# chenxuhao/GraphMiner

Hardware: AMD Instinct MI355X
Metric: million edges processed/sec + total match count (higher is better)
Workload: dtype int32 (vertex ids, offsets; uint64 counts); 1 GPU; tc: triangle counting, LiveJournal stand-in; graph=rmat_s22_ef10_seed42, nv=4194304, ne_sym=81171116, tasks=40585558, max_degree=777, parallelism=task-chunk round-robin x1, replicated CSR

## Files before the change

### graphminer_amd/csrc/gm_graph.hip

```cpp
#include "gm_host.h"
#include <unordered_map>
#include "gm_scan.h"
#include "gm_setops.h"
using namespace gm;

thread_local std::string g_last_error;
thread_local TempPool *g_temp_pool = nullptr;

namespace {
std::mutex g_opt_mu;
std::list<std::pair<std::string, std::string>> g_opts;
}
const char *gm_opt(const char *name) {
  if (!name) return nullptr;
  {
    std::lock_guard<std::mutex> lk(g_opt_mu);
    for (const auto &kv : g_opts)
      if (kv.first == name) return kv.second.c_str();
  }
#ifdef GM_DEVEL
  return getenv(name);
#else
  return nullptr;
#endif
// ... 165 lines not shown
  *n = 0;
  int c = 0;
  hipError_t e = hipGetDeviceCount(&c);
  if (e != hipSuccess) return hip_fail(e, "hipGetDeviceCount", __FILE__, __LINE__);
  *n = c;
  return c > 0 ? GM_OK : GM_ERR_NO_DEVICE;
}

extern "C" int gm_graph_setup_times(const gm_graph *g, gm_setup_times *out) {
  if (!g || !out) return GM_ERR_INVALID;
  *out = g->setup;
  for (const gm_graph *r : {g->dag_cache, g->relabel_cache[0], g->relabel_cache[1], g->relabel_cache[2]})
    if (r) {
      gm_setup_times t;
      const int rc = gm_graph_setup_times(r, &t);
      if (rc) return rc;
      out->orient_ms += t.orient_ms;
      out->table_ms += t.table_ms;
      out->bitmap_ms += t.bitmap_ms;
      out->relabel_ms += t.relabel_ms;
      out->other_ms += t.other_ms;
    }
  return GM_OK;
}
extern "C" void gm_graph_free(gm_graph *g) {
  if (!g) return;
  if (g->dag_cache) gm_graph_free(g->dag_cache);
  g->dag_cache = nullptr;
  for (auto &r : g->relabel_cache) {
    if (r) gm_graph_free(r);
    r = nullptr;
  }
  (void)hipSetDevice(g->device);
  free_tables(g);
  for (auto &b : g->bitmap_sets) {
    if (b.d_bitmaps) dev_free(b.d_bitmaps);
    if (b.d_row_slot) dev_free(b.d_row_slot);
  }
  if (g->d_rp) dev_free(g->d_rp);
  if (g->d_rp64) dev_free(g->d_rp64);
  if (g->own_col && g->d_col) dev_free(g->d_col);
  if (g->d_edesc) dev_free(g->d_edesc);
  if (g->d_symdeg) dev_free(g->d_symdeg);
  if (g->d_trp) dev_free(g->d_trp);
  if (g->d_tdesc) dev_free(g->d_tdesc);
  if (g->d_tedge) dev_free(g->d_tedge);
  for (void *q : {(void *)g->d_emoff, (void *)g->d_tmoff, (void *)g->d_smask, (void *)g->d_sup_far_rows})
    if (q) dev_free(q);
  if (g->d_long_rows) dev_free(g->d_long_rows);
  if (g->d_long_prefix) dev_free(g->d_long_prefix);
  if (g->d_colk) dev_free(g->d_colk);
  if (g->d_tdesck) dev_free(g->d_tdesck);
  if (g->d_kst) dev_free(g->d_kst);
  for (void *q : {(void *)g->d_kst_et, (void *)g->d_tedgel, (void *)g->d_kst2, (void *)g->d_tdescl2})
    if (q) dev_free(q);
  if (g->d_kst_rp) dev_free(g->d_kst_rp);
  if (g->d_trpl) dev_free(g->d_trpl);
  if (g->d_tdescl) dev_free(g->d_tdescl);
  if (g->d_sup) dev_free(g->d_sup);
  for (void *q : {(void *)g->d_w5sup, (void *)g->d_w5ed, (void *)g->d_w5deg, (void *)g->d_w5tv2, (void *)g->d_w5out})
    if (q) dev_free(q);
  for (void *q : {(void *)g->d_s6e1, (void *)g->d_wrect_mask, (void *)g->d_wrect_tasks})
    if (q) dev_free(q);
  for (void *q : {(void *)g->d_newid, (void *)g->d_lsup, (void *)g->d_lent, (void *)g->d_lrev, (void *)g->d_lmark, (void *)g->d_lfront, (void *)g->d_ltruss,
                  (void *)g->d_lcnt, (void *)g->d_list_off})
    if (q) dev_free(q);
  free_clique_plans(g);
  if (g->d_wide_mat) dev_free(g->d_wide_mat);
  if (g->d_wide_sorted) dev_free(g->d_wide_sorted);
  if (g->d_wide_queue) dev_free(g->d_wide_queue);
  for (auto &st_ : g->aux_stream) if (st_) (void)hipStreamDestroy(st_);
  for (auto &ev_ : g->aux_done) if (ev_) (void)hipEventDestroy(ev_);
  if (g->pool.base) dev_free(g->pool.base);
  if (g->d_counters) dev_free(g->d_counters);
  if (g->d_scratch) dev_free(g->d_scratch);
  if (g->d_core) dev_free(g->d_core);
  for (void *q : {(void *)g->d_cg_tri, (void *)g->d_cg_rowbase, (void *)g->d_cg_bid, (void *)g->d_cg_blk})
    if (q) dev_free(q);
  if (g->d_csym) dev_free(g->d_csym);
  if (g->d_cfirst) dev_free(g->d_cfirst);
  if (g->d_idx0) dev_free(g->d_idx0);
  if (g->d_wblock_prefix) dev_free(g->d_wblock_prefix);
  if (g->d_house_prefix) dev_free(g->d_house_prefix);
  if (g->d_pent_touched) dev_free(g->d_pent_touched);
  if (g->d_house_t) dev_free(g->d_house_t);
  if (g->d_house_tlt) dev_free(g->d_house_tlt);
  if (g->d_house_tasks) dev_free(g->d_house_tasks);
  if (g->d_house_acc) dev_free(g->d_house_acc);
  if (g->d_house_touched) dev_free(g->d_house_touched);
  if (g->d_house_bnd) dev_free(g->d_house_bnd);
  if (g->d_house_lds_tasks) dev_free(g->d_house_lds_tasks);
  if (g->d_house_cut_tasks) dev_free(g->d_house_cut_tasks);
  if (g->d_rect_tasks) dev_free(g->d_rect_tasks);
  if (g->d_rect_bnd) dev_free(g->d_rect_bnd);
  if (g->d_rect_lds_tasks) dev_free(g->d_rect_lds_tasks);
  if (g->d_rect_cut_tasks) dev_free(g->d_rect_cut_tasks);
  if (g->d_rect_acc) dev_free(g->d_rect_acc);
  for (auto &pr : g->ev)
    for (auto &e : pr)
      if (e) (void)hipEventDestroy(e);
  const bool last = g->counted && dev_handle_died(g->device);
  delete g;
  if (last) big_cache_trim();
}

int finish_handle(gm_graph *g) {
  if (!g->counted) {
// ... 971 lines not shown
```

### graphminer_amd/csrc/gm_host.h

```cpp
#pragma once
#include "../../include/graphminer_amd.h"
#include "gm_mine.h"
#include "gm_setops.h"

#include <algorithm>
#include <chrono>
#include <cstdio>
#include <cstring>
#include <list>
#include <mutex>
#include <string>
#include <thread>
#include <vector>

using namespace gm;

extern thread_local std::string g_last_error;
extern thread_local int g_last_hip_error;
int hip_fail(hipError_t e, const char *what, const char *file, int line);
#define HIP_TRY(call)                                              \
  do {                                                             \
    hipError_t _e = (call);                                        \
    if (_e != hipSuccess) return hip_fail(_e, #call, __FILE__, __LINE__); \
  } while (0)
// ... 150 lines not shown
struct CliquePlan {
  int rank = 0, world = 1, policy = 0, target = 0, order_which = 1;
  int stage = 1024;
  bool topo = false;
  ChunkTable *tabN = nullptr;
  long long n_first = 0, n_step = 1, n_count = 0;
  const int *d_order = nullptr;
  std::vector<int> verts;
  int *d_verts = nullptr;
  unsigned long long *d_slot_base = nullptr;
  int *d_mcls_slots = nullptr;
  int4 *d_mcls_rec = nullptr;
  int core_base = -1;
  std::vector<CliqueRound> rounds;
  unsigned long long wide_edges = 0;
};

struct BitmapSet {
  int min_deg = 0;
  RowFilter rf;
  unsigned *d_bitmaps = nullptr;
  int *d_row_slot = nullptr;
  size_t n = 0;
  unsigned long long words = 0;
};

struct gm_graph {
  int device = 0;
  int nv = 0;
  long long ne = 0;
  int max_deg = 0;
  int *d_rp = nullptr;
  long long *d_rp64 = nullptr;
  int *d_col = nullptr;
  bool own_col = true;
  int *d_symdeg = nullptr;
  int2 *d_edesc = nullptr;
  int *d_trp = nullptr;
  int2 *d_tdesc = nullptr;
  int *d_tedge = nullptr;
  int *d_colk = nullptr;
  int2 *d_tdesck = nullptr;
  unsigned long long n_inline_keys = 0;
  unsigned *d_kst = nullptr;
  int kst_state = 0;
  int n_long_tasks = 0;
  int *d_kst_rp = nullptr;
  int *d_trpl = nullptr;
  int2 *d_tdescl = nullptr;
  int2 *d_kst_et = nullptr;
  int *d_tedgel = nullptr;
  unsigned *d_kst2 = nullptr;
  int2 *d_tdescl2 = nullptr;
  int kst_lmax = 0;
  int *d_long_rows = nullptr;
  long long *d_long_prefix = nullptr;
  int n_long_rows = -1;
  long long long_edges = 0;
  unsigned *d_sup = nullptr;
  unsigned *d_w5sup = nullptr, *d_w5ed = nullptr;
  int *d_w5deg = nullptr;
  unsigned long long *d_w5tv2 = nullptr, *d_w5out = nullptr;
  bool w5_tri = false, w5_vert = false;
  unsigned *d_s6e1 = nullptr;
  unsigned long long *d_wrect_mask = nullptr;
  int2 *d_wrect_tasks = nullptr;
  unsigned long long n_wrect_tasks = 0;
  int wrect_range = 0, wrect_grp = 1;
  bool wrect_ready = false;
  int *d_newid = nullptr;
  unsigned *d_lsup = nullptr;
  unsigned *d_lent = nullptr;
  int *d_lrev = nullptr;
  bool lrev_ready = false;
  unsigned char *d_lmark = nullptr;
  int *d_lfront = nullptr;
  unsigned *d_ltruss = nullptr;
  unsigned *d_lcnt = nullptr;
  unsigned long long *d_list_off = nullptr;
  unsigned long long list_total = 0;
  bool list_ready = false;
  unsigned *d_emoff = nullptr, *d_tmoff = nullptr;
  unsigned long long *d_smask = nullptr;
  unsigned long long smask_words = 0;
  int *d_sup_far_rows = nullptr;
  int n_sup_far_rows = 0;
  int smask_min_tail = 0;
  int smask_state = 0;
  std::vector<int> h_rp;
  std::list<ChunkTable> tables;
  unsigned long long *d_counters = nullptr;
  unsigned *d_scratch = nullptr;
  size_t scratch_bytes = 0;
  static constexpr int kEvRing = 64;
  hipEvent_t ev[kEvRing][4] = {};
  bool ev_corner[kEvRing] = {};
  unsigned long long ev_launches = 0;
  int cu_count = 256;
  gm_graph *dag_cache = nullptr;
  gm_graph *relabel_cache[3] = {nullptr, nullptr, nullptr};
  int sorted_state = 0;
  int topo_state = 0;
  unsigned long long giant_edges = ~0ull;
  double tri_per_edge = -1.0;
  double mean_sq_deg = -1.0;
  bool topo_relabel_failed = false;
// ... 201 lines not shown
```

### graphminer_amd/csrc/gm_launch.hip

```cpp
#include "gm_host.h"

using namespace gm;

enum FinMode : int { FIN_COPY = 0, FIN_MOTIF3 = 1, FIN_MOTIF3_FORMULA = 2, FIN_RAW4 = 3, FIN_HALF_SIGNED = 4 };

__host__ __device__ static inline int finalize_math(int mode, unsigned long long base, const unsigned long long *c, unsigned long long *out) {
  if (mode == FIN_MOTIF3) {
    out[0] = c[2] - c[0];
    out[1] = c[1];
  } else if (mode == FIN_MOTIF3_FORMULA) {
    out[0] = base - 3ull * c[0];
    out[1] = c[0];
  } else if (mode == FIN_RAW4) {
    out[0] = c[0]; out[1] = c[1]; out[2] = c[2]; out[3] = c[3];
  } else if (mode == FIN_HALF_SIGNED) {
    out[0] = (unsigned long long)((long long)c[0] >> 1);
  } else {
    out[0] = c[0];
  }
  return mode == FIN_RAW4 ? 4 : (mode == FIN_MOTIF3 || mode == FIN_MOTIF3_FORMULA) ? 2 : 1;
}

__global__ void finalize_kernel(int mode, unsigned long long base, const unsigned long long *__restrict__ c,
                                unsigned long long *__restrict__ out) {
// ... 314 lines not shown
    q.count = (int)so->n;
    q.order = so->d;
    r.my_edges += so->edges;
    return GM_OK;
  }
  if (la->policy == GM_PART_VERTEX) {
    if (int rcv = table_host_views(g, tb)) return rcv;
    const long long vlo = (long long)g->nv * rank / world, vhi = (long long)g->nv * (rank + 1) / world;
    auto first_chunk_at = [&](long long v) {
      long long lo = 0, hi = n;
      while (lo < hi) {
        const long long mid = (lo + hi) / 2;
        if (tb->first_vertex[(size_t)mid] < v) lo = mid + 1; else hi = mid;
      }
      return lo;
    };
    first = first_chunk_at(vlo);
    count = first_chunk_at(vhi) - first;
  } else {
    gm_partition((int64_t)n, rank, world, la->policy, (int64_t *)&first, (int64_t *)&step, (int64_t *)&count);
  }
  q.first = (int)first;
  q.step = (int)step;
  q.count = (int)count;
  if (first == 0 && step == 1 && count == n) { r.my_edges += tb->total_edges; return GM_OK; }
  if (int rcv = table_host_views(g, tb)) return rcv;
  if (step == 1) r.my_edges += tb->edge_prefix[first + count] - tb->edge_prefix[first];
  else for (long long j = first; j < n; j += step) {
    const size_t c = lpt ? (size_t)tb->order[which][(size_t)j] : (size_t)j;
    r.my_edges += tb->edge_prefix[c + 1] - tb->edge_prefix[c];
  }
  return GM_OK;
}

static int fill_mine_params(PatternRun &r, int k) {
  gm_graph *g = r.ctx.g;
  const gm_launch *la = &r.ctx.la;
  const PatternPlan &pl = r.pl;
  MineParams &p = r.p;
  memset(&p, 0, sizeof p);
  p.g = graph_view(g);
  if (int rc = ensure_edesc(g)) return rc;
  p.g.edesc = g->d_edesc;
  if (pl.use_tct) {
    p.g.trp = g->d_trp;
    p.g.tdesc = g->d_tdesc;
    p.g.tedge = pl.support ? g->d_tedge : nullptr;
    if (pl.sup_masks) {
      p.g.tmoff = g->d_tmoff;
      p.smask = g->d_smask;
    }
    if (pl.use_kst && pl.support) {
      p.g.kst = g->d_kst2 ? g->d_kst2 : g->d_kst;
      p.g.kst_rp = g->d_kst_rp;
      p.g.kst_et = g->d_kst_et;
      p.g.trp = g->d_trpl;
      p.g.tdesc = g->d_tdescl2 ? g->d_tdescl2 : g->d_tdescl;
      p.g.tedge = g->d_tedgel;
    } else if (pl.use_kst) {
      p.g.kst = g->d_kst;
      p.g.kst_rp = g->d_kst_rp;
      p.g.trp = g->d_trpl;
      p.g.tdesc = g->d_tdescl;
    } else if (!pl.support && g->d_colk && g->d_tdesck && !(la->tune[6] & GM_T6_NO_KEYSTREAM)) {
      p.g.col = g->d_colk;
      p.g.tdesc = g->d_tdesck;
    }
  }
  if (int rc = take_share(r, pl.tab, p)) return rc;
  p.grab = la->tune[1] > 0 ? la->tune[1] : 1;
  if (la->tune[1] <= 0 && pl.use_tct && !pl.support && p.count >= 8ll * (long long)g->cu_count * (long long)(pl.tct_stage <= kStageCap ? 6 : 4)) p.grab = 2;
  p.cost_x_step = la->tune[2] > 0 ? la->tune[2] - 1 : 1;
  p.cost_y_step = la->tune[3] > 0 ? la->tune[3] - 1 : 6;
  p.cost_x_base = (la->tune[7] & 255) > 0 ? ((la->tune[7] >> 4) & 15) : 2;
  p.cost_y_base = (la->tune[7] & 255) > 0 ? (la->tune[7] & 15) : 2;
  p.cost_y_bitmap = la->tune[7] >> 8;
  p.k = k;
  p.flags = (la->tune[5] == 1) ? 1 : 0;
  p.flags |= (la->tune[6] & GM_T6_KERNEL_FLAGS_MASK) << 1;
  if (la->tune[6] & GM_T6_HROW_MUL32) p.flags |= 1 << 23;
  if (la->tune[6] & GM_T6_HSET_FALLBACK) p.flags |= 1 << 22;
  if (la->tune[6] & GM_T6_KCLIQUE_ANY_WIDTH) p.flags |= 1 << 20;
  p.counters = g->d_counters;
  p.queue = queue_word(g, QW_MAIN);
  return GM_OK;
}

static int prepare_scratch(PatternRun &r, int k) {
  gm_graph *g = r.ctx.g;
  const gm_launch *la = &r.ctx.la;
  const PatternPlan &pl = r.pl;
  MineParams &p = r.p;
  const size_t lds = mine_lds_bytes(pl.pat);
  r.per_cu = (int)std::max<size_t>(1, std::min<size_t>(8, (160 * 1024) / lds));
  if (la->tune[4] > 0) r.per_cu = la->tune[4];
  r.want = ((long long)p.count + (long long)p.grab - 1) / (long long)p.grab;
  r.grid = grid_for(r.want, g->cu_count, r.per_cu);
  if (pl.clique && pl.tab->max_bit_words > 0) {
    const unsigned long long region = pl.tab->max_bit_words + 4096ull;
    const int plist = (g->max_deg + 64) & ~63;
    const unsigned long long slot_words = (pl.pat == PAT_CLIQUEK) ? (unsigned long long)(k - 2) * (region + (unsigned long long)plist) : pl.tab->max_bit_words;
    p.scratch_region = region;
    p.scratch_plist = plist;
    {
      size_t free_b = 0, total_b = 0;
      (void)hipMemGetInfo(&free_b, &total_b);
      const unsigned long long budget = (unsigned long long)(free_b + g->scratch_bytes) / 2ull;
      const unsigned long long fit = budget / std::max<unsigned long long>(slot_words * sizeof(unsigned), 1ull);
      if (fit == 0) {
// ... 2047 lines not shown
```

### graphminer_amd/csrc/gm_mine.h

```cpp
#pragma once
#include <hip/hip_runtime.h>
#include <stdint.h>
#include <stdlib.h>

const char *gm_opt(const char *name);
inline const char *gm_sweep_env(const char *name) {
#ifdef GM_DEVEL
  return getenv(name);
#else
  (void)name;
  return nullptr;
#endif
}

namespace gm {

constexpr int kWavesPerBlock = 4;
constexpr int kStageCap = 1024;
#ifndef GM_STAGE_WIDE
#define GM_STAGE_WIDE 3072
#endif
constexpr int kStageCapWide = GM_STAGE_WIDE;
constexpr int kStageCapMid = 8191;
constexpr int kStageCapBig = 24576;
constexpr int kMaxChunkVerts = 256;
constexpr int kMarkWindow = 512;
#ifndef GM_TILES
#define GM_TILES 2
#endif
#define GM_TILES_DEFAULT GM_TILES
#ifndef GM_FILTER_LOG2
#define GM_FILTER_LOG2 15
#endif
constexpr int kFilterLog2 = GM_FILTER_LOG2;
constexpr int kFilterBits = 1 << kFilterLog2;
constexpr int kFilterWords = kFilterBits / 32;
constexpr int kQueueCap = 64 * (GM_TILES_DEFAULT + 1);
#ifndef GM_BIT_WORDS
#define GM_BIT_WORDS 2048
#endif
constexpr int kBitWords = GM_BIT_WORDS;
static_assert(GM_BIT_WORDS >= 2048 && GM_BIT_WORDS % 64 == 0, "rows of up to 2048 columns (stride 64) need 32 of them in one LDS group / tile");

constexpr int kSplitBatchMinKeys = 2048;
#ifndef GM_SPLIT_BATCH
#define GM_SPLIT_BATCH 16
#endif
constexpr int kSplitBatch = GM_SPLIT_BATCH;
struct ChunkRec {
  int u_begin, u_end, e_begin, e_end;
  int part, nparts;
  int batch, pad_;
};

struct GraphView {
  int nv;
  int ne;
  const int *rp;
  const int *col;
  const int2 *edesc = nullptr;
  const int *trp = nullptr;
  const int2 *tdesc = nullptr;
  const int *tedge = nullptr;
  const unsigned *tmoff = nullptr;
  const unsigned *kst = nullptr;
  const int *kst_rp = nullptr;
  const int2 *kst_et = nullptr;
};

#ifndef GM_LONG_LIST
#define GM_LONG_LIST 192
#endif
constexpr int kLongList = GM_LONG_LIST;
constexpr unsigned kNoMask = 0xffffffffu;
#ifndef GM_SUP_MASK_MIN_TAIL
#define GM_SUP_MASK_MIN_TAIL 2
#endif
constexpr int kSupMaskMinTail = GM_SUP_MASK_MIN_TAIL;
constexpr int kSupMaskSpare = 3;

enum Pattern : int { PAT_TC = 0, PAT_DIAMOND = 1, PAT_MOTIF3 = 2, PAT_CLIQUE4 = 3, PAT_CLIQUEK = 4 ,
                     PAT_MOTIF4E = 5 ,
                     PAT_DAGSTATS = 6 ,
                     PAT_SUPPORT = 7 ,
                     PAT_SUPPORT_PART = 8 ,
                     PAT_CLIQUEK_DEEP = 9 ,
                     PAT_WTRI = 10  };

#ifndef GM_PROBE_COST
#define GM_PROBE_COST 1
#endif
constexpr int kProbeCost = GM_PROBE_COST;
#ifndef GM_MID_PROBE_COST
#define GM_MID_PROBE_COST 1
#endif
constexpr int kMidProbeCost = GM_MID_PROBE_COST;
constexpr int kMidRowMax = 16384;
__host__ __device__ inline bool sym_hosts(int a, int b, int u, int v, int stage_cap) {
  const bool u_longer = (a > b) || (a == b && u > v);
  const int dl = u_longer ? a : b, ds = u_longer ? b : a;
  const int k = (dl <= kMidRowMax) ? kMidProbeCost : kProbeCost;
  const bool shorter_hosts = dl > stage_cap && ds <= stage_cap && (long long)dl < (long long)k * ds;
  return u_longer != shorter_hosts;
}

constexpr int kStageCapClique = 1024;
constexpr int stage_cap_of(int pat) {
  return (pat == PAT_DIAMOND || pat == PAT_MOTIF3 || pat == PAT_MOTIF4E) ? kStageCapWide
         : (pat == PAT_CLIQUE4 || pat == PAT_CLIQUEK || pat == PAT_CLIQUEK_DEEP) ? kStageCapClique : kStageCap;
}

struct MineParams {
  GraphView g;
  const ChunkRec *chunks;
  const int *chunk_slot;
  const int *order;
  unsigned long long *chunk_ticks;
  const unsigned *bitmaps;
  unsigned long long bitmap_words;
  const int *row_slot;
  int first, step, count;
  int grab;
  unsigned *queue;
  unsigned long long *counters;
  unsigned *scratch;
  unsigned long long scratch_words;
// ... 460 lines not shown
```

### graphminer_amd/csrc/gm_tables.hip

```cpp
#include "gm_host.h"
#include "gm_scan.h"
using namespace gm;

static void free_table(ChunkTable &t) {
  if (t.d) dev_free(t.d);
  if (t.d_slot) dev_free(t.d_slot);
  if (t.d_row_slot && t.own_bitmaps) dev_free(t.d_row_slot);
  for (int i = 0; i < 2; ++i) if (t.d_order[i]) dev_free(t.d_order[i]);
  if (t.d_bitmaps && t.own_bitmaps) dev_free(t.d_bitmaps);
  if (t.d_edges) dev_free(t.d_edges);
  if (t.d_firstv) dev_free(t.d_firstv);
  if (t.d_cost) dev_free(t.d_cost);
  for (auto &sh : t.shares)
    if (sh.d) dev_free(sh.d);
  t.shares.clear();
  t.d_edges = t.d_firstv = nullptr; t.d_cost = nullptr;
  t.d = nullptr; t.d_slot = nullptr; t.d_row_slot = nullptr; t.d_order[0] = t.d_order[1] = nullptr; t.d_bitmaps = nullptr;
}
void free_tables(gm_graph *g) {
  for (auto &t : g->tables) free_table(t);
  g->tables.clear();
}

constexpr int kTableBlock = 512;
// ... 947 lines not shown
}
__global__ __launch_bounds__(256) void kst_unpack_kernel(int nv, const unsigned long long *__restrict__ cnt, unsigned long long *__restrict__ keys, int *__restrict__ longs) {
  const int v = blockIdx.x * blockDim.x + threadIdx.x;
  if (v > nv) return;
  const unsigned long long c = v < nv ? cnt[v] : 0ull;
  keys[v] = c & 0xffffffffull;
  longs[v] = (int)(c >> 32);
}
__global__ __launch_bounds__(256) void kst_narrow_kernel(int nv, const unsigned long long *__restrict__ in, int *__restrict__ out) {
  const int v = blockIdx.x * blockDim.x + threadIdx.x;
  if (v <= nv) out[v] = (int)in[v];
}

constexpr double kTcCoreMinDensity = 0.03;
static int tc_core_size(gm_graph *g, const char *env = "GM_TC_CORE_H", bool blocks_only = false) {
  long long want = kTcCoreHDefault;
  bool forced = false;
  if (const char *e = gm_opt(env)) { want = atoll(e); forced = true; }
  if (want <= 0 || g->nv < 64) return 0;
  if (ensure_core_bitmap(g) != GM_OK || g->core_state != 1) return 0;
  const long long cap = std::min<long long>((long long)g->core_h, (long long)kCtcMaxH);
  auto aligned = [&](long long h) {
    const long long off = ((long long)g->core_h - h + 31) / 32 * 32;
    return off >= g->core_h ? 0ll : (long long)g->core_h - off;
  };
  if (forced) {
    const long long h = aligned(std::min(want, cap));
    return (int)((blocks_only && h % 512 != 0) ? 0 : h);
  }
  for (long long h = cap; h >= 1024; h >>= 1) {
    if ((long long)g->nv < 4 * h) continue;
    int e0 = 0;
    if (hipMemcpy(&e0, g->d_rp + (g->nv - h), sizeof(int), hipMemcpyDeviceToHost) != hipSuccess) { (void)hipGetLastError(); return 0; }
    const double rho = (double)(g->ne - (long long)e0) / (0.5 * (double)h * (double)h);
    if (rho >= kTcCoreMinDensity && !(blocks_only && aligned(h) % 512 != 0)) return (int)aligned(h);
  }
  return 0;
}
int ensure_keystream(gm_graph *g, bool edges, bool *built, bool allow_core) {
  auto have = [&]() { return g->d_kst_rp != nullptr && (!edges || g->d_kst_et != nullptr); };
  *built = have();
  if (*built || g->kst_state == 2 || g->ne == 0) return GM_OK;
  if (edges && g->d_kst_rp != nullptr && g->kst_skip_from < g->nv) return GM_OK;
  {
    const int rc = ensure_edesc(g);
    if (rc) return rc;
  }
  const int tc_h = (allow_core && !edges && g->d_kst_rp == nullptr) ? tc_core_size(g) : 0;
  std::lock_guard<std::mutex> lk(g->mu);
  *built = have();
  if (*built || g->kst_state == 2) return GM_OK;
  if (edges && g->d_kst_rp != nullptr && g->kst_skip_from < g->nv) return GM_OK;
  const bool second = g->d_kst_rp != nullptr;
  int lmax = second ? g->kst_lmax : GM_TC_INLINE_MAX_DEFAULT;
  if (!second) {
    if (const char *e = gm_sweep_env("GM_TC_INLINE_MAX")) lmax = atoi(e);
    if (!keystream_possible(g) || lmax < 4) {
      g->kst_state = 2;
      return GM_OK;
    }
  }
  SetupTimer timer;
  HIP_TRY(hipSetDevice(g->device));
  const size_t nv1 = (size_t)g->nv + 1;
  PoolScope pool(g);
  ScanTemp tmp;
  bool topo = false;
  {
    const int rc = graph_is_topological(g, &topo);
    if (rc) return rc;
    if (gm_sweep_env("GM_TC_NO_TRIM")) topo = false;
  }
  DevBuf<unsigned long long> cnt, keys, keyoff;
  DevBuf<int> longs;
  HIP_TRY(cnt.alloc(nv1));
  HIP_TRY(keys.alloc(nv1));
  HIP_TRY(keyoff.alloc(nv1));
  HIP_TRY(longs.alloc(nv1));
  int win_count = kHubWin, win_place = 2048, per_cu_count = topo ? 8 : 64, per_cu_place = topo ? 16 : 64;
  if (const char *e = gm_sweep_env("GM_KST_HUB_WIN")) win_count = win_place = std::max(0, std::min(atoi(e), kHubWin));
  if (const char *e = gm_sweep_env("GM_KST_WG_PER_CU")) per_cu_count = per_cu_place = std::max(1, atoi(e));
  const long long blocks_count = std::min<long long>(((long long)g->nv * 8 + 255) / 256, (long long)g->cu_count * per_cu_count);
  const long long blocks_place = std::min<long long>(((long long)g->nv * 8 + 255) / 256, (long long)g->cu_count * per_cu_place);
  TaskWalk tw;
  tw.nv = g->nv; tw.stage_max = kTctStageMax; tw.topo = topo ? 1 : 0;
  tw.rp = g->d_rp; tw.col = g->d_col; tw.edesc = g->d_edesc;
  const int skip_from = (!second && topo && tc_h > 0) ? g->nv - tc_h : 0x7fffffff;
  tw.skip_from = skip_from;
  long long core_edges = 0;
  if (skip_from < g->nv) {
    int e0 = 0;
    HIP_TRY(hipMemcpy(&e0, g->d_rp + skip_from, sizeof(int), hipMemcpyDeviceToHost));
    core_edges = g->ne - (long long)e0;
  }
  TaskWalk tw_count = tw, tw_place = tw;
  tw_count.hub0 = topo ? std::max(0, g->nv - win_count) : g->nv;
  tw_place.hub0 = topo ? std::max(0, g->nv - win_place) : g->nv;
  int *krp = second ? g->d_kst_rp : nullptr, *trpl = second ? g->d_trpl : nullptr;
  unsigned *kst = nullptr;
  int2 *tdl = nullptr;
  KstEdges ed{nullptr, nullptr};
  auto fail = [&](hipError_t e, const char *what) {
    for (void *q : {second ? nullptr : (void *)krp, second ? nullptr : (void *)trpl, (void *)kst, (void *)tdl, (void *)ed.kst_et, (void *)ed.tedgel})
      if (q) dev_free(q);
    return hip_fail(e, what, __FILE__, __LINE__);
  };
  hipError_t e = hipSuccess;
  if (!second && ((e = dev_malloc(&krp, sizeof(int) * nv1)) != hipSuccess || (e = dev_malloc(&trpl, sizeof(int) * nv1)) != hipSuccess)) return fail(e, "hipMalloc(key stream offsets)");
  unsigned long long total = second ? g->n_inline_keys : 0, key_limit = 0x7fffff00ull;
  if (const char *e = gm_opt("GM_KST_MAX_KEYS")) key_limit = std::min<unsigned long long>(key_limit, (unsigned long long)std::max(1ll, atoll(e)));
  int nlong = second ? g->n_long_tasks : 0;
  while (!second) {
    if ((e = hipMemsetAsync(cnt.p, 0, sizeof(unsigned long long) * nv1, 0)) != hipSuccess) return fail(e, "hipMemsetAsync");
    if (win_count <= 2048) hipLaunchKernelGGL((kst_rows_kernel<false, 2048, false>), dim3((unsigned)blocks_count), dim3(256), 0, 0, tw_count, lmax, cnt.p, nullptr, nullptr, nullptr, nullptr, ed);
    else hipLaunchKernelGGL((kst_rows_kernel<false, kHubWin, false>), dim3((unsigned)blocks_count), dim3(256), 0, 0, tw_count, lmax, cnt.p, nullptr, nullptr, nullptr, nullptr, ed);
    hipLaunchKernelGGL(kst_unpack_kernel, dim3((unsigned)((nv1 + 255) / 256)), dim3(256), 0, 0, g->nv, cnt.p, keys.p, longs.p);
    if ((e = dev_exclusive_sum(tmp, keys.p, keyoff.p, nv1)) != hipSuccess) return fail(e, "ExclusiveSum");
    if ((e = dev_exclusive_sum(tmp, longs.p, trpl, nv1)) != hipSuccess) return fail(e, "ExclusiveSum");
    if ((e = hipMemcpy(&total, keyoff.p + g->nv, 8, hipMemcpyDeviceToHost)) != hipSuccess) return fail(e, "hipMemcpy");
    if ((e = hipMemcpy(&nlong, trpl + g->nv, sizeof(int), hipMemcpyDeviceToHost)) != hipSuccess) return fail(e, "hipMemcpy");
    if (total < key_limit) break;
    lmax >>= 1;
    if (lmax < 4) {
      dev_free(krp);
      dev_free(trpl);
      g->kst_state = 2;
      return GM_OK;
    }
  }
  setup_trace("key stream: count pass + scans");
  if (!second) hipLaunchKernelGGL(kst_narrow_kernel, dim3((unsigned)((nv1 + 255) / 256)), dim3(256), 0, 0, g->nv, keyoff.p, krp);
  const size_t nk = (size_t)std::max<unsigned long long>(total, 1), nl = (size_t)std::max(nlong, 1);
  if ((e = dev_malloc(&kst, sizeof(unsigned) * nk)) != hipSuccess) return fail(e, "hipMalloc(key stream)");
  if ((e = dev_malloc(&tdl, sizeof(int2) * nl)) != hipSuccess) return fail(e, "hipMalloc(long lists)");
  if (edges && ((e = dev_malloc(&ed.kst_et, sizeof(int2) * nk)) != hipSuccess || (e = dev_malloc(&ed.tedgel, sizeof(int) * nl)) != hipSuccess))
    return fail(e, "hipMalloc(key stream entries)");
  if ((e = hipMemsetAsync(cnt.p, 0, sizeof(unsigned long long) * nv1, 0)) != hipSuccess) return fail(e, "hipMemsetAsync");
  const dim3 pg((unsigned)blocks_place), pb(256);
  if (edges) {
    if (win_place <= 2048) hipLaunchKernelGGL((kst_rows_kernel<true, 2048, true>), pg, pb, 0, 0, tw_place, lmax, cnt.p, krp, trpl, kst, tdl, ed);
    else hipLaunchKernelGGL((kst_rows_kernel<true, kHubWin, true>), pg, pb, 0, 0, tw_place, lmax, cnt.p, krp, trpl, kst, tdl, ed);
  } else {
    if (win_place <= 2048) hipLaunchKernelGGL((kst_rows_kernel<true, 2048, false>), pg, pb, 0, 0, tw_place, lmax, cnt.p, krp, trpl, kst, tdl, ed);
    else hipLaunchKernelGGL((kst_rows_kernel<true, kHubWin, false>), pg, pb, 0, 0, tw_place, lmax, cnt.p, krp, trpl, kst, tdl, ed);
  }
  if ((e = hipGetLastError()) != hipSuccess || (e = hipDeviceSynchronize()) != hipSuccess) return fail(e, "kst_rows_kernel");
  setup_trace("key stream: place pass");
  if (second) {
    g->d_kst2 = kst;
    g->d_tdescl2 = tdl;
  } else {
    g->d_kst = kst;
    g->d_trpl = trpl;
    g->d_tdescl = tdl;
    g->n_inline_keys = total;
    g->n_long_tasks = nlong;
    g->kst_lmax = lmax;
    if (skip_from < g->nv) {
      g->tc_core_edges = core_edges;
      g->tc_core_h = g->nv - skip_from;
      g->kst_skip_from = skip_from;
    }
  }
  if (edges) {
    g->d_tedgel = ed.tedgel;
    g->d_kst_et = ed.kst_et;
  }
  if (!second) g->d_kst_rp = krp;
  g->setup.table_ms += timer.ms();
  *built = true;
  return GM_OK;
}

int ensure_tasklists(gm_graph *g, bool ) {
  if (__atomic_load_n(&g->d_tdesc, __ATOMIC_ACQUIRE) || g->ne == 0) return GM_OK;
  {
    const int rc = ensure_edesc(g);
    if (rc) return rc;
  }
  const int tl_h = g->max_deg <= kTctStageMax ? tc_core_size(g, "GM_SUP_CORE_H", true) : 0;
  std::lock_guard<std::mutex> lk(g->mu);
  if (g->d_tdesc) return GM_OK;
  SetupTimer timer;
  HIP_TRY(hipSetDevice(g->device));
  const size_t ne = (size_t)g->ne, nv1 = (size_t)g->nv + 1;
  PoolScope pool(g);
  DevBuf<int> cnt;
  ScanTemp tmp;
  bool topo = false;
  {
    const int rc = graph_is_topological(g, &topo);
    if (rc) return rc;
    if (gm_sweep_env("GM_TC_NO_TRIM")) topo = false;
  }
  setup_trace("tasks: sorted / topological check");
  HIP_TRY(cnt.alloc(nv1));
  HIP_TRY(hipMemsetAsync(cnt.p, 0, sizeof(int) * nv1, 0));
  const long long blocks = std::min<long long>(((long long)g->nv * 8 + 255) / 256, (long long)g->cu_count * (topo ? 8 : 64));
  TaskWalk tw;
  tw.nv = g->nv; tw.stage_max = kTctStageMax; tw.topo = topo ? 1 : 0;
  tw.hub0 = topo ? std::max(0, g->nv - kHubWin) : g->nv;
  tw.rp = g->d_rp; tw.col = g->d_col; tw.edesc = g->d_edesc;
  const int tl_skip = (topo && tl_h > 0) ? g->nv - tl_h : 0x7fffffff;
// ... 1050 lines not shown
```

### graphminer_amd/csrc/gm_tch.hip

```cpp
#include <type_traits>
#include "gm_flat.h"

namespace gm {

#ifndef GM_TCH_TILES
#define GM_TCH_TILES 4
#endif
constexpr int kTchTiles = GM_TCH_TILES;
#ifndef GM_TCH_TILES_SMALL
#define GM_TCH_TILES_SMALL 2
#endif
constexpr int kTchTilesSmall = GM_TCH_TILES_SMALL;
constexpr int kTchFlatTilesSmall = 4, kTchFlatTilesBig = 8;

#ifndef GM_TCH_LONG_LIST
#define GM_TCH_LONG_LIST 384
#endif
constexpr int kTchLongList = GM_TCH_LONG_LIST;

constexpr int kTchOvfCap = 128;
constexpr unsigned kTchEmpty = 0xffffffffu, kTchMarker = 0xfffffffeu;
constexpr unsigned kTchMul = 0x9E3779B1u;

template <int BITWIN>
struct alignas(16) TchWave {
  int2 desc[GM_WAVE];
  unsigned bits[BITWIN / 32 + 8];
};

#ifndef GM_TCH_WAVES_BIG
#define GM_TCH_WAVES_BIG 4
#endif
#ifndef GM_TCH_MIN_WG_BIG
#define GM_TCH_MIN_WG_BIG 4
#endif
template <int STAGE>
constexpr int tch_waves() { return STAGE <= 1024 ? kWavesPerBlock : GM_TCH_WAVES_BIG; }
template <int STAGE>
struct alignas(16) TchLds {
  uint4 table[STAGE];
  int rpl[kMaxChunkVerts + 1];
  int trpl[kMaxChunkVerts + 1];
  static constexpr int kBitWindow = STAGE <= 1024 ? 8192 : 4096;
  TchWave<kBitWindow> w[tch_waves<STAGE>()];
  int ovf_key[kTchOvfCap];
  int ovf_salt[kTchOvfCap];
  int n_ovf;
  int next_batch;
  unsigned queue_pos;
  int next_group;
};
static_assert(kTchOvfCap == 2 * GM_WAVE, "the surplus list is scanned two entries per lane");

template <int STAGE>
struct TchHash {
  static constexpr int LB = STAGE == 1024 ? 10 : 11;
  static_assert((1 << LB) == STAGE, "one bucket per stage entry");
  static constexpr unsigned kMask = (unsigned)(STAGE - 1) << 4;
  static __device__ __forceinline__ unsigned bucket(int x, unsigned s) { return ((((unsigned)x * kTchMul) >> (28 - LB)) & kMask) ^ s; }
  static __device__ __forceinline__ unsigned salt(int local_row) { return (((unsigned)local_row * 37u) & (unsigned)(STAGE - 1)) << 4; }
  static __device__ __forceinline__ int row_of(unsigned s) { return (int)(((s >> 4) * 941u) & (unsigned)(STAGE - 1)); }
};

__device__ __forceinline__ int tch_local_row(const int *rpl, const int nvl, const int e) {
  int lo = 0, hi = nvl - 1;
  while (lo < hi) {
    const int mid = (lo + hi + 1) >> 1;
    if (rpl[mid] <= e) lo = mid; else hi = mid - 1;
  }
  return lo;
}
// ... 403 lines not shown
```

### graphminer_amd/csrc/gm_tools.hip

```cpp
#include "gm_host.h"
#include "gm_setops.h"
#include "gm_flat.h"
using namespace gm;

__global__ __launch_bounds__(256) void setop_kernel(int op, long long npairs, const int *__restrict__ vals,
                                                    const long long *__restrict__ ab, const long long *__restrict__ ae,
                                                    const long long *__restrict__ bb, const long long *__restrict__ be,
                                                    const int *__restrict__ upper, const int *__restrict__ skip,
                                                    unsigned *__restrict__ out_num, int *__restrict__ out_vals) {
  const int lane = threadIdx.x & 63;
  const long long wave = ((long long)blockIdx.x * blockDim.x + threadIdx.x) >> 6;
  const long long nwaves = ((long long)gridDim.x * blockDim.x) >> 6;
  for (long long i = wave; i < npairs; i += nwaves) {
    const int *A = vals + ab[i];
    const int *B = vals + bb[i];
    const int a = (int)(ae[i] - ab[i]), b = (int)(be[i] - bb[i]);
    const int up = upper ? upper[i] : 0x7fffffff;
    const int sk = skip ? skip[i] : -1;
    int *O = out_vals ? out_vals + ab[i] : nullptr;
    unsigned r = 0;
    switch (op) {
      case GM_OP_INTERSECT_NUM: r = (unsigned)wave_sum((int)wave_intersect_num(A, a, B, b)); break;
      case GM_OP_INTERSECT_NUM_UPPER: r = (unsigned)wave_sum((int)wave_intersect_num_upper(A, a, B, b, up)); break;
      case GM_OP_INTERSECT_SET: r = (unsigned)wave_intersect_set(A, a, B, b, O); break;
// ... 56 lines not shown
    }
  }
}

extern "C" int gm_rmat_keys(int scale, int64_t n_edges, uint64_t seed, uint64_t *d_keys, void *stream) {
  if (scale < 1 || scale > 30 || n_edges < 0 || !d_keys) return GM_ERR_INVALID;
  if (n_edges == 0) return GM_OK;
  const long long blocks = std::min<long long>((n_edges + 255) / 256, 65536);
  hipLaunchKernelGGL(rmat_kernel, dim3((unsigned)blocks), dim3(256), 0, (hipStream_t)stream, scale, (long long)n_edges,
                     (unsigned long long)seed, (unsigned long long *)d_keys);
  HIP_TRY(hipGetLastError());
  return GM_OK;
}

__global__ __launch_bounds__(256) void calib_stream_kernel(const int *__restrict__ buf, long long n, unsigned long long *out) {
  const long long stride = (long long)gridDim.x * blockDim.x;
  unsigned long long acc = 0;
  for (long long i = (long long)blockIdx.x * blockDim.x + threadIdx.x; i < n; i += stride) acc += (unsigned)buf[i];
  acc = wave_sum_u64(acc);
  if ((threadIdx.x & 63) == 0 && acc) atomicAdd(out, acc);
}

extern "C" int gm_calib_stream(const int32_t *d_buf, int64_t n, uint64_t *d_out, void *stream) {
  if (!d_buf || !d_out || n < 0) return GM_ERR_INVALID;
  hipLaunchKernelGGL(calib_stream_kernel, dim3(256 * 8), dim3(256), 0, (hipStream_t)stream, d_buf, (long long)n,
                     (unsigned long long *)d_out);
  HIP_TRY(hipGetLastError());
  return GM_OK;
}

typedef int gm_v4i __attribute__((ext_vector_type(4)));
__global__ __launch_bounds__(256) void stream_ceiling_kernel(const gm_v4i *__restrict__ buf, long long n4, unsigned long long *out) {
  const long long stride = (long long)gridDim.x * blockDim.x;
  long long i = (long long)blockIdx.x * blockDim.x + threadIdx.x;
  gm_v4i acc = {0, 0, 0, 0};
  for (; i + 3 * stride < n4; i += 4 * stride) {
    const gm_v4i a = __builtin_nontemporal_load(buf + i), b = __builtin_nontemporal_load(buf + i + stride);
    const gm_v4i c = __builtin_nontemporal_load(buf + i + 2 * stride), d = __builtin_nontemporal_load(buf + i + 3 * stride);
    acc ^= a ^ b ^ c ^ d;
  }
  for (; i < n4; i += stride) acc ^= buf[i];
  const unsigned long long s = wave_sum_u64((unsigned long long)(unsigned)(acc.x ^ acc.y ^ acc.z ^ acc.w));
  if ((threadIdx.x & 63) == 0 && s) atomicAdd(out, s);
}

extern "C" int gm_constant(const char *name, int64_t *value) {
  if (!name || !value) return GM_ERR_INVALID;
  static const struct { const char *name; long long v; } tab[] = {
      {"tct_stage_max", kTctStageMax},       {"topo_min_mean_row", kTopoMinMeanRow}, {"motif_trim_min_list", kMotifTrimMinList},
      {"cb_min_deg", kCbMinDeg},             {"cb_max_deg", kCbMaxDeg},               {"long_list", kLongList},
      {"stage_cap", kStageCap},              {"default_chunk", kDefaultChunk},        {"mma_words_small", kMmaWordsS},
      {"mma_words_big", kMmaWordsL},         {"core_h_default", kCoreHDefault},  {"wide_min_words", kWideMinWordsDefault},
              {"wide_max_deg", kWideMaxDeg},           {"bit_words", kBitWords},
  };
  for (const auto &e : tab)
    if (strcmp(e.name, name) == 0) {
      *value = e.v;
      return GM_OK;
    }
  g_last_error = std::string("gm_constant: unknown name '") + name + "'";
  return GM_ERR_INVALID;
}

extern "C" int gm_stream_ceiling(const int32_t *d_buf, int64_t n, uint64_t *d_out, void *stream) {
  if (!d_buf || !d_out || n < 0 || ((uintptr_t)d_buf & 15)) return GM_ERR_INVALID;
  int dev = 0, cus = 256;
  hipDeviceProp_t prop;
  if (hipGetDevice(&dev) == hipSuccess && hipGetDeviceProperties(&prop, dev) == hipSuccess && prop.multiProcessorCount > 0) cus = prop.multiProcessorCount;
  hipLaunchKernelGGL(stream_ceiling_kernel, dim3((unsigned)(cus * 8)), dim3(256), 0, (hipStream_t)stream, (const gm_v4i *)d_buf,
                     (long long)(n / 4), (unsigned long long *)d_out);
  HIP_TRY(hipGetLastError());
  return GM_OK;
}

__global__ void selftest_kernel(int *out) {
  __shared__ int lds[64];
  const int lane = threadIdx.x;
  const int x = (lane * 7 + 3) % 11;
  out[lane] = wave_incl_scan_add(x);
  const int y = (lane % 9 == 0) ? lane + 1 : 0;
  out[64 + lane] = wave_incl_scan_max(y);
  const unsigned long long m = __ballot((lane % 3) == 1);
  out[128 + lane] = rank_below(m);
  out[192 + lane] = lane_id();
  lds[lane] = lane * 3;
  wave_sync();
  int pos;
  const bool f = contains(&lds[0], 64, lane * 2, &pos);
  out[256 + lane] = f ? pos : -1;
  out[320 + lane] = lower_bound(&lds[0], 64, lane * 2);
  out[384 + lane] = (int)wave_sum_u64((unsigned long long)lane + (1ull << 33));
  out[448 + lane] = (int)(wave_sum_u64((unsigned long long)lane + (1ull << 33)) >> 32);
}

extern "C" int gm_selftest(int device, int *n_fail) {
  if (n_fail) *n_fail = -1;
  HIP_TRY(hipSetDevice(device));
  int *d = nullptr;
  HIP_TRY(dev_malloc(&d, sizeof(int) * 512));
  hipLaunchKernelGGL(selftest_kernel, dim3(1), dim3(64), 0, 0, d);
  int h[512];
  hipError_t e = hipMemcpy(h, d, sizeof h, hipMemcpyDeviceToHost);
  dev_free(d);
  if (e != hipSuccess) return hip_fail(e, "selftest", __FILE__, __LINE__);
  int bad = 0, acc = 0, mx = 0, rk = 0;
  for (int l = 0; l < 64; ++l) {
// ... 276 lines not shown
```

Baseline: 23930 Medges/s.

## Widen first key-stream set threshold for TC and give second set own offsets

For the non-edge key-stream build, the first set now takes neighbor lists up to a larger default length (kTcStreamMax, overridable via GM_TC_STREAM_MAX), so more triangle-counting lists are read inline from the compact key stream instead of through the long-list path. When the first set's threshold exceeds the inline default, the second (support) set can no longer reuse the first set's row offsets, so it allocates its own kst_rp2/trpl2 arrays and the launch code picks them up. This trades a larger key-stream buffer and extra setup memory for fewer long-list lookups during counting.

```diff
diff --git a/graphminer_amd/csrc/gm_graph.hip b/graphminer_amd/csrc/gm_graph.hip
--- a/graphminer_amd/csrc/gm_graph.hip
+++ b/graphminer_amd/csrc/gm_graph.hip
@@ -241,7 +241,7 @@
   if (g->d_colk) dev_free(g->d_colk);
   if (g->d_tdesck) dev_free(g->d_tdesck);
   if (g->d_kst) dev_free(g->d_kst);
-  for (void *q : {(void *)g->d_kst_et, (void *)g->d_tedgel, (void *)g->d_kst2, (void *)g->d_tdescl2})
+  for (void *q : {(void *)g->d_kst_et, (void *)g->d_tedgel, (void *)g->d_kst2, (void *)g->d_tdescl2, (void *)g->d_kst_rp2, (void *)g->d_trpl2})
     if (q) dev_free(q);
   if (g->d_kst_rp) dev_free(g->d_kst_rp);
   if (g->d_trpl) dev_free(g->d_trpl);
diff --git a/graphminer_amd/csrc/gm_host.h b/graphminer_amd/csrc/gm_host.h
--- a/graphminer_amd/csrc/gm_host.h
+++ b/graphminer_amd/csrc/gm_host.h
@@ -226,6 +226,8 @@
   int *d_tedgel = nullptr;
   unsigned *d_kst2 = nullptr;
   int2 *d_tdescl2 = nullptr;
+  int *d_kst_rp2 = nullptr;
+  int *d_trpl2 = nullptr;
   int kst_lmax = 0;
   int *d_long_rows = nullptr;
   long long *d_long_prefix = nullptr;
diff --git a/graphminer_amd/csrc/gm_launch.hip b/graphminer_amd/csrc/gm_launch.hip
--- a/graphminer_amd/csrc/gm_launch.hip
+++ b/graphminer_amd/csrc/gm_launch.hip
@@ -390,9 +390,9 @@
     }
     if (pl.use_kst && pl.support) {
       p.g.kst = g->d_kst2 ? g->d_kst2 : g->d_kst;
-      p.g.kst_rp = g->d_kst_rp;
+      p.g.kst_rp = g->d_kst_rp2 ? g->d_kst_rp2 : g->d_kst_rp;
       p.g.kst_et = g->d_kst_et;
-      p.g.trp = g->d_trpl;
+      p.g.trp = g->d_trpl2 ? g->d_trpl2 : g->d_trpl;
       p.g.tdesc = g->d_tdescl2 ? g->d_tdescl2 : g->d_tdescl;
       p.g.tedge = g->d_tedgel;
     } else if (pl.use_kst) {
diff --git a/graphminer_amd/csrc/gm_mine.h b/graphminer_amd/csrc/gm_mine.h
--- a/graphminer_amd/csrc/gm_mine.h
+++ b/graphminer_amd/csrc/gm_mine.h
@@ -72,6 +72,15 @@
 #define GM_LONG_LIST 192
 #endif
 constexpr int kLongList = GM_LONG_LIST;
+#ifndef GM_TCH_LONG_LIST
+#define GM_TCH_LONG_LIST 384
+#endif
+constexpr int kTchLongList = GM_TCH_LONG_LIST;
+#ifndef GM_TC_STREAM_MAX_DEFAULT
+#define GM_TC_STREAM_MAX_DEFAULT 32
+#endif
+constexpr int kTcStreamMax = GM_TC_STREAM_MAX_DEFAULT;
+static_assert(kTcStreamMax >= 4 && kTcStreamMax < kTchLongList, "the stream holds lists below tch_kernel's one-at-a-time threshold");
 constexpr unsigned kNoMask = 0xffffffffu;
 #ifndef GM_SUP_MASK_MIN_TAIL
 #define GM_SUP_MASK_MIN_TAIL 2
diff --git a/graphminer_amd/csrc/gm_tables.hip b/graphminer_amd/csrc/gm_tables.hip
--- a/graphminer_amd/csrc/gm_tables.hip
+++ b/graphminer_amd/csrc/gm_tables.hip
@@ -1023,13 +1023,17 @@
   if (*built || g->kst_state == 2) return GM_OK;
   if (edges && g->d_kst_rp != nullptr && g->kst_skip_from < g->nv) return GM_OK;
   const bool second = g->d_kst_rp != nullptr;
-  int lmax = second ? g->kst_lmax : GM_TC_INLINE_MAX_DEFAULT;
+  const bool share = second && g->kst_lmax <= GM_TC_INLINE_MAX_DEFAULT;
+  int lmax = share ? g->kst_lmax : ((edges || second) ? GM_TC_INLINE_MAX_DEFAULT : kTcStreamMax);
   if (!second) {
     if (const char *e = gm_sweep_env("GM_TC_INLINE_MAX")) lmax = atoi(e);
+    if (!edges)
+      if (const char *e = gm_opt("GM_TC_STREAM_MAX")) lmax = std::min(atoi(e), kTchLongList - 1);
     if (!keystream_possible(g) || lmax < 4) {
       g->kst_state = 2;
       return GM_OK;
     }
+    lmax = (int)std::min<unsigned long long>((unsigned long long)lmax, 0xffffffffull / (unsigned long long)std::max(g->nv, 1));
   }
   SetupTimer timer;
   HIP_TRY(hipSetDevice(g->device));
@@ -1067,21 +1071,21 @@
   TaskWalk tw_count = tw, tw_place = tw;
   tw_count.hub0 = topo ? std::max(0, g->nv - win_count) : g->nv;
   tw_place.hub0 = topo ? std::max(0, g->nv - win_place) : g->nv;
-  int *krp = second ? g->d_kst_rp : nullptr, *trpl = second ? g->d_trpl : nullptr;
+  int *krp = share ? g->d_kst_rp : nullptr, *trpl = share ? g->d_trpl : nullptr;
   unsigned *kst = nullptr;
   int2 *tdl = nullptr;
   KstEdges ed{nullptr, nullptr};
   auto fail = [&](hipError_t e, const char *what) {
-    for (void *q : {second ? nullptr : (void *)krp, second ? nullptr : (void *)trpl, (void *)kst, (void *)tdl, (void *)ed.kst_et, (void *)ed.tedgel})
+    for (void *q : {share ? nullptr : (void *)krp, share ? nullptr : (void *)trpl, (void *)kst, (void *)tdl, (void *)ed.kst_et, (void *)ed.tedgel})
       if (q) dev_free(q);
     return hip_fail(e, what, __FILE__, __LINE__);
   };
   hipError_t e = hipSuccess;
-  if (!second && ((e = dev_malloc(&krp, sizeof(int) * nv1)) != hipSuccess || (e = dev_malloc(&trpl, sizeof(int) * nv1)) != hipSuccess)) return fail(e, "hipMalloc(key stream offsets)");
-  unsigned long long total = second ? g->n_inline_keys : 0, key_limit = 0x7fffff00ull;
+  if (!share && ((e = dev_malloc(&krp, sizeof(int) * nv1)) != hipSuccess || (e = dev_malloc(&trpl, sizeof(int) * nv1)) != hipSuccess)) return fail(e, "hipMalloc(key stream offsets)");
+  unsigned long long total = share ? g->n_inline_keys : 0, key_limit = 0x7fffff00ull;
   if (const char *e = gm_opt("GM_KST_MAX_KEYS")) key_limit = std::min<unsigned long long>(key_limit, (unsigned long long)std::max(1ll, atoll(e)));
-  int nlong = second ? g->n_long_tasks : 0;
-  while (!second) {
+  int nlong = share ? g->n_long_tasks : 0;
+  while (!share) {
     if ((e = hipMemsetAsync(cnt.p, 0, sizeof(unsigned long long) * nv1, 0)) != hipSuccess) return fail(e, "hipMemsetAsync");
     if (win_count <= 2048) hipLaunchKernelGGL((kst_rows_kernel<false, 2048, false>), dim3((unsigned)blocks_count), dim3(256), 0, 0, tw_count, lmax, cnt.p, nullptr, nullptr, nullptr, nullptr, ed);
     else hipLaunchKernelGGL((kst_rows_kernel<false, kHubWin, false>), dim3((unsigned)blocks_count), dim3(256), 0, 0, tw_count, lmax, cnt.p, nullptr, nullptr, nullptr, nullptr, ed);
@@ -1100,7 +1104,8 @@
     }
   }
   setup_trace("key stream: count pass + scans");
-  if (!second) hipLaunchKernelGGL(kst_narrow_kernel, dim3((unsigned)((nv1 + 255) / 256)), dim3(256), 0, 0, g->nv, keyoff.p, krp);
+  if (gm_sweep_env("GM_TABLE_INFO")) fprintf(stderr, "[key stream] set %d: lists of <= %d keys, %llu keys (%.1f MB), %d longer lists\n", second ? 2 : 1, lmax, total, 4e-6 * (double)total, nlong);
+  if (!share) hipLaunchKernelGGL(kst_narrow_kernel, dim3((unsigned)((nv1 + 255) / 256)), dim3(256), 0, 0, g->nv, keyoff.p, krp);
   const size_t nk = (size_t)std::max<unsigned long long>(total, 1), nl = (size_t)std::max(nlong, 1);
   if ((e = dev_malloc(&kst, sizeof(unsigned) * nk)) != hipSuccess) return fail(e, "hipMalloc(key stream)");
   if ((e = dev_malloc(&tdl, sizeof(int2) * nl)) != hipSuccess) return fail(e, "hipMalloc(long lists)");
@@ -1120,6 +1125,10 @@
   if (second) {
     g->d_kst2 = kst;
     g->d_tdescl2 = tdl;
+    if (!share) {
+      g->d_kst_rp2 = krp;
+      g->d_trpl2 = trpl;
+    }
   } else {
     g->d_kst = kst;
     g->d_trpl = trpl;
diff --git a/graphminer_amd/csrc/gm_tch.hip b/graphminer_amd/csrc/gm_tch.hip
--- a/graphminer_amd/csrc/gm_tch.hip
+++ b/graphminer_amd/csrc/gm_tch.hip
@@ -13,10 +13,6 @@
 constexpr int kTchTilesSmall = GM_TCH_TILES_SMALL;
 constexpr int kTchFlatTilesSmall = 4, kTchFlatTilesBig = 8;
 
-#ifndef GM_TCH_LONG_LIST
-#define GM_TCH_LONG_LIST 384
-#endif
-constexpr int kTchLongList = GM_TCH_LONG_LIST;
 
 constexpr int kTchOvfCap = 128;
 constexpr unsigned kTchEmpty = 0xffffffffu, kTchMarker = 0xfffffffeu;
diff --git a/graphminer_amd/csrc/gm_tools.hip b/graphminer_amd/csrc/gm_tools.hip
--- a/graphminer_amd/csrc/gm_tools.hip
+++ b/graphminer_amd/csrc/gm_tools.hip
@@ -132,6 +132,7 @@
       {"stage_cap", kStageCap},              {"default_chunk", kDefaultChunk},        {"mma_words_small", kMmaWordsS},
       {"mma_words_big", kMmaWordsL},         {"core_h_default", kCoreHDefault},  {"wide_min_words", kWideMinWordsDefault},
               {"wide_max_deg", kWideMaxDeg},           {"bit_words", kBitWords},
+      {"tch_long_list", kTchLongList},       {"tc_stream_max", kTcStreamMax},
   };
   for (const auto &e : tab)
     if (strcmp(e.name, name) == 0) {
```

Result: no change. 23920 Medges/s (median of 2 runs) (-0.0%).
